# MILVLG/mmnas

Hardware: AMD Instinct MI355X
Metric: supernet fwd+bwd steps/sec (VQA arch, bs=64) (higher is better)
Workload: dtype f32 (bf16x6 split-operand MFMA, fp32 accumulate); 1 GPU; Net_Search supernet WEIGHT step: sample + fwd + BCE(sum) + bwd (+ gradient all-reduce), HSIZE 256, B=64/GPU, 100x2048 regions + 14 tokens, dropout 0.1 (search_vqa.py:279-292; BASELINE configs[2]); global_batch=64, parallelism=dp1, grad_allreduce=none, rccl_ranks=1, rank_id_sum_ok=True, lstm_fallback=False, dp_rows=1, dp_buckets=3, optimizer_in_step=False, gemm_split=6, hip_force_dev_kernarg=1

## Files before the change

include/mmnas_hip.h:

```cpp
#ifndef MMNAS_HIP_H
#define MMNAS_HIP_H

#include <stddef.h>
#include <stdint.h>

#ifdef __cplusplus
extern "C" {
#endif

#define MMNAS_ABI_VERSION 1

enum {
  MMNAS_OK = 0,
  MMNAS_E_SHAPE = -1,
  MMNAS_E_ARG = -2,
  MMNAS_E_LAUNCH = -3
};

enum {
  MMNAS_F_NORM = 1,
  MMNAS_F_RESIDUAL = 2,
  MMNAS_F_MASK = 4,
  MMNAS_F_REL = 8,
  MMNAS_F_SELF = 16,
// ... 290 lines not shown
  void* arena;
  float* x_out; float* y_out;
  const float* dx_out; const float* dy_out;
  float* dx_in; float* dy_in;
  int use_side_stream, reserved;
  void* const* marks;
  int mixed, gate_width;
  const float* gate;
  float* dgate;
  const int* y_off;
  const int* y_tile_off;
  int Ny, y_ntiles;
  const int* x_off;
  int Nx, reserved3;
} mmnas_chain;
int mmnas_chain_plan(const mmnas_chain* c, size_t* arena_bytes);
int mmnas_chain_fwd(const mmnas_chain* c, void* stream);
int mmnas_chain_bwd(const mmnas_chain* c, void* stream);
int mmnas_chain_join(void* main_stream, void* waiting_stream);
int mmnas_set_chain_overlap(int on);
int mmnas_set_wgrad_live(int on);
int mmnas_wgrad_live_table_ints(int M);
int mmnas_wgrad_live_table(const float* dy, const unsigned char* mask, int M, int d, int* tab, void* stream);

typedef struct mmnas_attflat_side {
  int S, reserved;
  const float* x; const uint8_t* mask;
  const float* W1; const float* b1; const float* W2; const float* b2; const float* Wm; const float* bm;
  float* dW1; float* db1; float* dW2; float* db2; float* dWm; float* dbm;
  uint64_t seed;
  float* dx;
  const int* off;
  int M, reserved2;
} mmnas_attflat_side;
typedef struct mmnas_head {
  int B, d, MID, G, OUT, ANS, flags, reserved;
  float drop_p, eps;
  mmnas_attflat_side sx, sy;
  const float* ln_a; const float* ln_b; float* dln_a; float* dln_b;
  const float* Wp; const float* bp; float* dWp; float* dbp;
  float* logits;
  const float* dlogits;
  void* arena;
} mmnas_head;
int mmnas_head_plan(const mmnas_head* hd, size_t* arena_bytes);
int mmnas_head_fwd(const mmnas_head* hd, void* stream);
// ... 76 lines not shown
```

mmnas_amd/_lib.py:

```python
import ctypes as C
import logging
import os

import torch

from . import switches

_HERE = os.path.dirname(os.path.abspath(__file__))
LIB_PATH = os.environ.get(switches.LIB_PATH.name) or os.path.join(_HERE, 'lib', 'libmmnas_hip.so')

log = logging.getLogger('mmnas_amd')


def _launch_configuration():
    name = 'HIP_FORCE_DEV_KERNARG'
    if name in os.environ:
        return os.environ[name], 'inherited'
    if torch.cuda.is_initialized():
        log.warning('mmnas_amd was imported after HIP had initialised and %s is not set: kernel arguments go through host-visible '
                    'memory, the ~300 short launches of a step run 20-40 %% slower.  Export %s=1 or import mmnas / mmnas_amd '
                    'before the first CUDA call.', name, name)
        return None, 'unset_after_hip_init'
    os.environ[name] = '1'
    return '1', 'set_by_library'
# ... 164 lines not shown
    'mmnas_alpha_full_step_cost': (_i, [_fp] * 7 + [_i, _i, _f, _f, _f, _f, _f, _f, _f, _i, _i, _fp]),
    'mmnas_alpha_two_step_cost': (_i, [_fp] * 7 + [_i, _i, C.POINTER(C.c_int), _f, _f, _f, _f, _f, _f, _f, _i, _i, _fp]),
    'mmnas_embedding_bwd': (_i, [_fp, _fp, _fp, C.c_long, _i, C.c_long, _fp]),
    'mmnas_node_mix_fwd': (_i, [_fp, _fp, _fp, _i, _fp, _fp, _i, _i, _f, _fp]),
    'mmnas_node_mix_bwd': (_i, [_fp, _fp, _fp, _i, _fp, _fp, _fp, _i, _fp, _fp, _i, _i, _f, _fp]),
    'mmnas_node_mix_bwd_ln': (_i, [_fp, _fp, _fp, _i, _fp, _fp, _i, _fp, _fp, _fp, _fp, _fp, _fp, _fp, _fp, _f, _u64, _u32, _i, _i, _f, _fp]),
    'mmnas_embedding_bwd_det': (_i, [_fp, _fp, _fp, _fp, C.c_long, _i, C.c_long, _f, _fp]),
    'mmnas_embedding_bwd_det_ws_floats': (_sz, [C.c_long, _i]),
    'mmnas_rel_fused_supported': (_i, [_i, _i, _i]),
    'mmnas_rel_fused_fwd': (_i, [_fp, _fp, _fp, _fp, _fp, _fp, _i, _i, _i, _i, _i, _i, _fp]),
    'mmnas_rel_fused_bwd_ws_floats': (_sz, [_i, _i, _i]),
    'mmnas_rel_fused_bwd': (_i, [_fp, _fp, _fp, _fp, _fp, _fp, _fp, _fp, _fp, _fp, _fp, _i, _i, _i, _i, _i, _i, _fp]),
    'mmnas_rel_fused_fwd_ragged': (_i, [_fp, _fp, _fp, _fp, _fp, _fp, _i, _i, _i, _i, _i, _fp, _fp]),
    'mmnas_rel_fused_bwd_ragged': (_i, [_fp] * 11 + [_i, _i, _i, _i, _i, _fp, _fp, _i, _fp]),
    'mmnas_rel_multi_supported': (_i, [_i, _i, _i]),
    'mmnas_rel_multi_bwd_ws_floats': (_sz, [_i, _i]),
    'mmnas_rel_multi_fwd': (_i, [C.POINTER(RelMulti), _fp]),
    'mmnas_rel_multi_bwd': (_i, [C.POINTER(RelMulti), _fp]),
    'mmnas_set_rel_hoist': (_i, [_i]),
    'mmnas_set_rel_keylimit': (_i, [_i]),
    'mmnas_set_wgrad_live': (_i, [_i]),
    'mmnas_wgrad_live_table_ints': (_i, [_i]),
    'mmnas_wgrad_live_table': (_i, [_fp, _fp, _i, _i, _fp, _fp]),
    'mmnas_set_guided_hoist': (_i, [_i]),
    'mmnas_set_rel_overlap': (_i, [_i]),
    'mmnas_mha_core_fwd': (_i, [C.POINTER(MhaDesc), _fp]),
    'mmnas_mha_core_bwd': (_i, [C.POINTER(MhaDesc), _fp]),
    'mmnas_mha_core_fwd_indexed': (_i, [C.POINTER(MhaDesc), _fp, _fp]),
    'mmnas_itm_pair_head': (_i, [_fp] * 11 + [C.c_long, _i, _i, _f, _fp]),
    'mmnas_rank_matrix': (_i, [_fp, _i, _i, C.c_long, _fp, _fp, _fp, _fp, _fp, _fp]),
    'mmnas_row_topk': (_i, [_fp, _i, _i, C.c_long, _i, _fp, _fp, _fp]),
    'mmnas_vgd_targets': (_i, [_fp, _fp, _fp, _i, _i, C.c_double, _i, _fp, _fp, _fp, _fp, _fp, _fp, _fp]),
    'mmnas_vgd_ground': (_i, [_fp] * 5 + [_i, _i, C.c_double] + [_fp] * 7),
    'mmnas_vqa_answer': (_i, [_fp, _i, _i, C.c_long, _fp, C.c_long, _i, _i] + [_fp] * 4 + [_i] + [_fp] * 5),
    'mmnas_vqa_accuracy': (_i, [_fp] * 4 + [_i] * 4 + [_fp, _fp, _fp]),
    'mmnas_vqa_answer_targets': (_i, [_fp, _i, _i, _i, _fp, _fp, _fp]),
    'mmnas_vgd_loss_fwd': (_i, [_fp] * 6 + [_i] * 6 + [C.c_double, C.c_double] + [_fp] * 5),
    'mmnas_itm_triplet_loss_fwd': (_i, [_fp, _fp, _fp, C.c_long, _i, _f, _i, _fp, _fp, _fp]),
    'mmnas_loss_grad_scale': (_i, [_fp, _fp, _fp, _sz, _fp]),
    'mmnas_vgd_head_supported': (_i, [_i, _i]),
    'mmnas_vgd_head_bwd_ws_floats': (_sz, [_i, _i, _i]),
    'mmnas_vgd_head_fwd': (_i, [_fp] * 12 + [_i, _i, _i, _f, _i, _fp]),
    'mmnas_vgd_head_bwd': (_i, [_fp] * 20 + [_i, _i, _i, _f, _i, _fp]),
    'mmnas_att_op_plan': (_i, [C.POINTER(AttOp), C.POINTER(Plan)]),
    'mmnas_att_op_fwd': (_i, [C.POINTER(AttOp), _fp]),
    'mmnas_att_op_bwd': (_i, [C.POINTER(AttOp), _fp]),
# ... 78 lines not shown
```

mmnas_amd/csrc/ops.hip:

```cpp
#include <string.h>
#include <functional>
#include <vector>
#include "common.h"

namespace mmnas {

static inline size_t al(size_t n) { return (n + 255) & ~(size_t)255; }
template <class Op> static inline bool drops(const Op* op) { return (op->flags & MMNAS_F_TRAIN) && op->drop_p > 0.f; }

struct Carver {
  char* base; size_t off;
  explicit Carver(void* p) : base((char*)p), off(0) {}
  float* take(size_t nfloats) { float* r = (float*)(base + off); off += al(nfloats * sizeof(float)); return r; }
};

static void gemm_init(mmnas_gemm_desc& g, int layout, int N, int K, int lda, int ldb, int ldc) {
  memset(&g, 0, sizeof(g));
  g.layout = layout; g.ngroups = 1; g.nseg = 1; g.N = N; g.K = K; g.lda = lda; g.ldb = ldb; g.ldc = ldc;
  g.alpha = 1.f; g.gate_scale = 1.f; g.split_k = 1;
}

struct AttLayout {
  size_t Mq, Mk;
  float *Q, *K, *V, *att, *stats, *z, *biasT;
// ... 723 lines not shown
    b.a.xq = in; b.a.xkv = self ? in : chain_x_final(c, L);
    b.a.dy = dy; b.a.dxq = dx;
    b.a.dxkv = self ? nullptr : chain_buf(c, L.dpre);
    b.a.drel = nullptr;
  } else { b.m.x = in; b.m.dy = dy; b.m.dx = dx; }
  return dx;
}
static int chain_run_fwd(const BoundOp& b, hipStream_t s, bool defer_ln, bool* ln_done, bool rel_ready, bool kv_ready) {
  return b.att ? att_fwd_impl(&b.a, s, defer_ln, ln_done, rel_ready, kv_ready) : mlp_fwd_impl(&b.m, s, defer_ln, ln_done);
}
static int chain_run_bwd(const BoundOp& b, hipStream_t s, SideQueue* sq, bool rel_defer, bool kv_defer, const AuxReduce* ln_pre = nullptr) {
  return b.att ? att_bwd_impl(&b.a, s, sq, !(b.a.flags & MMNAS_F_SELF), rel_defer, kv_defer, ln_pre, b.ktab) : mlp_bwd_impl(&b.m, s, sq, ln_pre, b.ktab);
}
static LnPlace chain_cand_view(const BoundOp& b, const float** z, const float** la, const float** lb) {
  LnPlace p = {false, false};
  if (b.att) p = att_ln_place(&b.a);
  if (!(b.flags() & MMNAS_F_NORM) || p.fwd) { *z = b.y; *la = nullptr; *lb = nullptr; }
  else if (b.att) { *z = b.al.z; *la = b.a.ln_a; *lb = b.a.ln_b; }
  else { *z = b.ml.z; *la = b.m.ln_a; *lb = b.m.ln_b; }
  return p;
}

constexpr int LIVE_MAX_ROWS = 8192;
int sk_workspace(hipStream_t st, float** ws, size_t* ws_floats, int** cnt, int* ncnt);
typedef unsigned u32x4_t __attribute__((ext_vector_type(4)));

__global__ void __launch_bounds__(256) wgrad_live_kernel(const float* __restrict__ dy, const uint8_t* __restrict__ mask, const int M, const int d,
                                                         int* __restrict__ tab, unsigned* __restrict__ bits, const int nwords, int* __restrict__ cnt) {
  __shared__ int s_last;
  const int tid = threadIdx.x, lane = tid & 63, wave = tid >> 6;
  const int w = blockIdx.x * 4 + wave;
  if (w < nwords) {
    const int r0 = w * 32;
    const int r = r0 + (lane & 31);
    const bool in = lane < 32 && r < M;
    const bool masked = in && mask[r] != 0;
    const unsigned need = (unsigned)__ballot(masked);
    unsigned live = (unsigned)__ballot(in && !masked);
    const __amdgpu_buffer_rsrc_t rs = __builtin_amdgcn_make_buffer_rsrc((void*)dy, 0, (unsigned)M * (unsigned)d * 4u, 0x00020000);
    for (int c0 = 0; c0 < d; c0 += 256) {
      const int col = c0 + lane * 4;
#pragma unroll
      for (int hb = 0; hb < 2; ++hb) {
        u32x4_t v[16];
#pragma unroll
        for (int i = 0; i < 16; ++i) {
          const int rr = hb * 16 + i;
          const bool ld = ((need >> rr) & 1u) != 0 && col < d;
          v[i] = __builtin_amdgcn_raw_buffer_load_b128(rs, ld ? (unsigned)((r0 + rr) * d + col) * 4u : ~0u, 0, 0);
        }
#pragma unroll
        for (int i = 0; i < 16; ++i) {
          const bool nz = ((v[i].x | v[i].y | v[i].z | v[i].w) & 0x7fffffffu) != 0;
          if (__ballot(nz) != 0) live |= 1u << (hb * 16 + i);
        }
      }
    }
    if (lane == 0) __hip_atomic_store(bits + w, live, __ATOMIC_RELAXED, __HIP_MEMORY_SCOPE_AGENT);
  }
  asm volatile("s_waitcnt vmcnt(0)" ::: "memory");
  __syncthreads();
  if (tid == 0) s_last = __hip_atomic_fetch_add(cnt, 1, __ATOMIC_RELAXED, __HIP_MEMORY_SCOPE_AGENT) == (int)gridDim.x - 1;
  __syncthreads();
  if (!s_last || wave != 0) return;
  if (lane == 0) __hip_atomic_store(cnt, 0, __ATOMIC_RELAXED, __HIP_MEMORY_SCOPE_AGENT);
  unsigned wd[4];
#pragma unroll
  for (int j = 0; j < 4; ++j) {
    const int i = 2 * lane + (j & 1) + 128 * (j >> 1);
    wd[j] = i < nwords ? __hip_atomic_load(bits + i, __ATOMIC_RELAXED, __HIP_MEMORY_SCOPE_AGENT) : 0u;
  }
  int count = 0, pos = 0;
  while (pos < M) {
    const int wi = pos >> 6, sl = wi & 63;
    const unsigned lo = wi < 64 ? __builtin_amdgcn_readlane(wd[0], sl) : __builtin_amdgcn_readlane(wd[2], sl);
    const unsigned hi = wi < 64 ? __builtin_amdgcn_readlane(wd[1], sl) : __builtin_amdgcn_readlane(wd[3], sl);
    const unsigned long long m = (((unsigned long long)hi << 32) | lo) >> (pos & 63);
    if (m == 0) { pos = (wi + 1) << 6; continue; }
    const int r = pos + __builtin_ctzll(m);
    if (lane == 0) tab[1 + count] = r;
    ++count;
    pos = r + 32;
  }
  if (lane == 0) tab[0] = count;
}

static int live_table_launch(const float* dy, const uint8_t* mask, int M, int d, int* tab, hipStream_t st) {
  const int nwords = cdiv(M, 32);
  float* ws; size_t wsf; int* cnt; int ncnt;
  const int rc = sk_workspace(st, &ws, &wsf, &cnt, &ncnt);
  if (rc) return rc;
  MMNAS_LAUNCH(wgrad_live_kernel, dim3(cdiv(nwords, 4)), dim3(256), 0, st, dy, mask, M, d, tab, (unsigned*)(tab + 1 + nwords), nwords, cnt + ncnt - 1);
  return check_launch("wgrad_live_table");
}
static bool live_table_fits(long M, int d) { return M > 0 && M <= LIVE_MAX_ROWS && d > 0 && d % 4 == 0 && (double)M * d * 4.0 < 4.0e9; }

struct SideCtx { hipStream_t side; hipStream_t enc; hipEvent_t ev[MMNAS_CHAIN_MAX_OPS + 2]; hipEvent_t ovl[4]; bool used; };
static std::mutex g_side_mu;
static std::map<std::pair<int, hipStream_t>, SideCtx> g_side;

static SideCtx* side_ctx(hipStream_t main, bool create) {
  int dev = 0;
  if (hipGetDevice(&dev) != hipSuccess) return nullptr;
  std::lock_guard<std::mutex> lk(g_side_mu);
  auto key = std::make_pair(dev, main);
  auto it = g_side.find(key);
  if (it == g_side.end()) {
// ... 207 lines not shown
  return chain_rel_fwd(RG, st, 0);
}
static int chain_rel_join(SideCtx* rsc, hipStream_t st) { return ev_fork(rsc->side, st, rsc->ovl[1]); }
static int chain_fwd_passthrough(const mmnas_chain* c, const ChainLayout& L, hipStream_t st) {
  const size_t nx = chain_rows_x(c) * c->d * sizeof(float), ny = chain_rows_y(c) * c->d * sizeof(float);
  if (L.last_x < 0 && hipMemcpyAsync(c->x_out, c->x_in, nx, hipMemcpyDeviceToDevice, st) != hipSuccess) return MMNAS_E_LAUNCH;
  if (L.last_y < 0 && hipMemcpyAsync(c->y_out, c->y_in, ny, hipMemcpyDeviceToDevice, st) != hipSuccess) return MMNAS_E_LAUNCH;
  return MMNAS_OK;
}

struct ChainBwd {
  const mmnas_chain* c; const ChainLayout* L;
  hipStream_t st;
  SideQueue* sq;
  RelGroups RG;
  GuidedSet GS;
  int G;
  float *dpre, *encdy;
  size_t ex;
  const float* enc_grad = nullptr;
  SideCtx* rel_bwd_side = nullptr;
  const int* ktab = nullptr;
};
static int chain_live_table(const mmnas_chain* c, const ChainLayout& L, hipStream_t st, const int** out) {
  *out = nullptr;
  if (!c->y_mask || c->y_off || L.first_y < 0 || !sw::wgrad_live.get() || !live_table_fits((long)c->B * c->Sy, c->d)) return MMNAS_OK;
  int* tab = (int*)chain_buf(c, L.ktab);
  const int rc = live_table_launch(c->dy_out, c->y_mask, c->B * c->Sy, c->d, tab, st);
  if (!rc) *out = tab;
  return rc;
}
static int chain_bwd_begin(ChainBwd& S, const mmnas_chain* c, const ChainLayout& L, hipStream_t st, SideQueue* sq, bool hoist) {
  S.c = c; S.L = &L; S.st = st; S.sq = sq;
  S.dpre = chain_buf(c, L.dpre); S.encdy = chain_buf(c, L.encdy);
  S.ex = chain_rows_x(c) * c->d;
  if (int r = chain_live_table(c, L, st, &S.ktab)) return r;
  if (hoist) chain_rel_groups(c, L, true, S.RG);
  chain_guided_set(c, true, hoist, S.GS);
  S.G = -1;
  for (int i = 0; i < c->n_ops && S.G < 0; ++i)
    if (S.GS.hoisted[i]) S.G = i;
  if (L.n_guided > S.GS.n && hipMemsetAsync(S.dpre, 0, S.ex * sizeof(float), st) != hipSuccess) return MMNAS_E_LAUNCH;
  return MMNAS_OK;
}
static int chain_enc_dy(ChainBwd& S, hipStream_t s, const float** out) {
  const mmnas_chain* c = S.c;
  MMNAS_REQUIRE(c->dx_out || S.L->n_guided, MMNAS_E_ARG, "chain_bwd: no gradient reaches the encoder (dx_out NULL, no guided operator)");
  if (S.enc_grad) { *out = S.enc_grad; return MMNAS_OK; }
  if (c->dx_out && S.L->n_guided) {
    const int r = mmnas_drop_add(c->dx_out, S.dpre, S.encdy, S.ex, 0.f, 0, 0, s);
// ... 292 lines not shown
    SideCtx* oc = side_ctx(st, true);
    MMNAS_REQUIRE(oc, MMNAS_E_LAUNCH, "chain_bwd: cannot create the encoder stream");
    for (int i = c->n_ops - 1; i >= G; --i)
      if ((rc = run(i, st, cur_dy, &cur_dy))) return rc;
    if ((rc = ev_fork(st, oc->enc, oc->ovl[2]))) return rc;
    const float* enc_dy = nullptr;
    if ((rc = chain_enc_dy(S, oc->enc, &enc_dy))) return rc;
    int ie = L.last_x, id = G - 1;
    while (ie >= L.first_x || id >= L.first_y) {
      if (ie >= L.first_x && (rc = run(ie--, oc->enc, enc_dy, &enc_dy))) return rc;
      if (id >= L.first_y && (rc = run(id--, st, cur_dy, &cur_dy))) return rc;
    }
    if ((rc = ev_fork(oc->enc, st, oc->ovl[3]))) return rc;
    if (c->marks)
      for (int i = 0; i < c->n_ops; ++i)
        if (c->marks[i] && hipEventRecord((hipEvent_t)c->marks[i], st) != hipSuccess) {
          set_error("chain_bwd: cannot record the mark event of operator %d", i);
          return MMNAS_E_LAUNCH;
        }
  }
  return chain_bwd_close(S, nullptr);
}

extern "C" int mmnas_chain_join(void* main_stream, void* waiting_stream) {
  SideCtx* sc = side_ctx((hipStream_t)main_stream, false);
  if (!sc || !sc->used) return MMNAS_OK;
  hipEvent_t e = sc->ev[MMNAS_CHAIN_MAX_OPS];
  if (hipEventRecord(e, sc->side) != hipSuccess || hipStreamWaitEvent((hipStream_t)waiting_stream, e, 0) != hipSuccess) {
    set_error("chain_join: event record / wait failed");
    return MMNAS_E_LAUNCH;
  }
  return MMNAS_OK;
}

namespace mmnas {

struct HeadSideLayout { float *h, *logit, *probs, *pooled, *dpooled, *dlog, *dh, *dxpool, *g1part; };
static inline int head_rows(const mmnas_head* hd, const mmnas_attflat_side& sd) { return sd.off ? sd.M : hd->B * sd.S; }
struct HeadLayout {
  HeadSideLayout s[2];
  float *xo, *sum, *xy, *dxy, *dsum, *lnws, *g1proj, *dlogT;
  size_t total;
};

static HeadLayout head_layout(const mmnas_head* hd) {
  HeadLayout L;
// ... 189 lines not shown
```

mmnas_amd/csrc/switches.h:

```cpp
#pragma once

namespace mmnas {

int env_int(const char* name, int dflt);

enum SwKind { sw_int, sw_bool, sw_exact1, sw_presence, sw_string };
enum SwPolicy { sw_once, sw_every_call, sw_reload };

struct Switch {
  const char* name;
  int dflt;
  SwKind kind;
  SwPolicy policy;
  const char* help;
  int value;
  int state;

  int get() { return state ? value : read(); }
  int read();
  int reload();
  int set(int v);
  int peek(int* source) const;
};

#define MMNAS_SWITCHES(X) \
   \
  X(chain_overlap, "MMNAS_CHAIN_OVERLAP", 0, bool, once, "language stream beside the leading image-stream operators (mmnas_set_chain_overlap); measured: no gain, DESIGN.md section 5") \
  X(head_overlap, "MMNAS_HEAD_OVERLAP", 0, bool, once, "the answer head's two AttFlat sides on two streams") \
  X(head_glimpse1, "MMNAS_HEAD_GLIMPSE1", 1, bool, every_call, "0: the head's one-glimpse logit layer as GEMM launches (A/B, tests); ops.py reads it too") \
  X(head_projt, "MMNAS_HEAD_PROJT", 1, bool, every_call, "0: the answer projection's gradients from the untransposed loss gradient") \
  X(rel_hoist, "MMNAS_REL_HOIST", 1, bool, once, "relation bias of all lazy-handle operators of a stream in one launch per direction (mmnas_set_rel_hoist); 0: one fused launch per operator (supernet step 4.54 -> 5.00 ms)") \
  X(rel_overlap, "MMNAS_REL_OVERLAP", 0, bool, once, "the image stream's relation launches on a second stream (mmnas_set_rel_overlap); measured slower, +2.5 % on the supernet step") \
  X(node_lnb, "MMNAS_NODE_LNB", 1, bool, once, "architecture step: the sampled candidate's LayerNorm backward inside the node's mix kernel (7.81 -> 7.72 ms, profiles/r06_node_lnb_ab.txt); 0: its own launch") \
  X(guided_hoist, "MMNAS_GUIDED_HOIST", 1, bool, once, "key / value projections of a chain's guided operators as grouped launches (mmnas_set_guided_hoist)") \
  X(rel_fwd_valu, "MMNAS_REL_FWD_VALU", 0, exact1, every_call, "1: a lone RelSelfAtt computes its bias with the per-operator fused kernel instead of the one-operator multi kernel (A/B)") \
  X(side_prio, "MMNAS_SIDE_PRIO", 1, bool, every_call, "0: the chains' extra streams without stream priorities (read when a stream pair is created)") \
  X(side_flush, "MMNAS_SIDE_FLUSH", 0, string, once, "op: side-stream parameter-gradient work released behind every operator instead of once per phase") \
  X(wgrad_live, "MMNAS_WGRAD_LIVE", 1, int, once, "image-stream weight gradients of a padded batch's chain reduce over the 32-row K-tiles that cover the live gradient rows only (mmnas_set_wgrad_live); 0: all B Sy rows") \
   \
  X(small_ops, "MMNAS_SMALL_OPS", 1, bool, once, "SelfAtt of <= 16 rows as one launch forward (mmnas_set_small_ops); 0: the general path") \
  X(small_bwd, "MMNAS_SMALL_BWD", 1, bool, once, "the same operators' backward as two launches (mmnas_set_small_bwd)") \
  X(small_ffn, "MMNAS_SMALL_FFN", 0, int, once, "FeedForward forward as one launch (mmnas_set_small_ffn): 1 four slices of 256 hidden units, 2 eight of 128; measured neutral (profiles/r05_small_ffn_ab.txt)") \
   \
  X(gemm_ln, "MMNAS_GEMM_LN", 0, exact1, once, "1: the merge / last FFN product and its LayerNorm as one row-panel launch (mmnas_set_gemm_ln); measured neutral, profiles/r06_ab.txt") \
  X(gemm_ln_minm, "MMNAS_GEMM_LN_MINM", 2048, int, once, "fewest rows for the row-panel kernel (read together with MMNAS_GEMM_LN)") \
  X(gemm_ln_maxk, "MMNAS_GEMM_LN_MAXK", 256, int, once, "largest K for the row-panel kernel (read together with MMNAS_GEMM_LN)") \
   \
  X(mha_nw, "MMNAS_MHA_NW", 4, int, every_call, "2: attention cores never use 4-wave workgroups (4-wave groups measured 7-15 % faster; the streaming forward always runs four)") \
  X(mha_stream_mink, "MMNAS_MHA_STREAM_MINK", 257, int, every_call, "fewest keys at which the attention forward streams the keys in blocks of 128 (1..257; more than 256 keys always stream; dense rows only)") \
  X(mha_pair, "MMNAS_MHA_PAIR", 1, bool, once, "0: two attention cores of one geometry as two launches (mixed chain)") \
  X(mha_bwd_fused, "MMNAS_MHA_BWD_FUSED", 1, bool, once, "0: the attention backward as separate dQ and dK / dV kernels (dense rows only)") \
  X(mha_fwd_b16, "MMNAS_MHA_FWD_B16", 1, bool, once, "0: attention forward (d_h = 64, 65..128 keys) on the fp32 MFMA kernels instead of split-bf16 operands (profiles/r06_attention_b16_ab.txt)") \
  X(mha_fwd_b16_two, "MMNAS_MHA_FWD_B16_TWO", 320, int, once, "more than this many (sample, head) pairs: the split-bf16 forward runs two per workgroup") \
  X(mha_bwd_b16, "MMNAS_MHA_BWD_B16", 1, bool, once, "0: attention backward (d_h = 64, 65..128 keys) on the fp32 MFMA kernels instead of split-bf16 operands (supernet step -1.6 % with both)") \
   \
  X(rel_multi_dbg, "MMNAS_REL_MULTI_DBG", 0, int, once, "timing experiments of a -DMMNAS_DBG_REL=1 build only (wrong results): 1 no stores, 2 no raw reloads, 4 no head-projection MFMAs") \
  X(rel_multi_wgs, "MMNAS_REL_MULTI_WGS", 3, int, once, "workgroups per CU of the multi-operator relation forward (tuning)") \
  X(rel_multi_yield, "MMNAS_REL_MULTI_YIELD", 0, int, once, "1 | 3: the multi-operator relation kernels' yield variants (tuning)") \
  X(rel_keylimit, "MMNAS_REL_KEYLIMIT", 1, int, once, "multi-operator relation kernels of a padded batch walk only the elements under keys up to each sample's last unmasked one (mmnas_set_rel_keylimit); 0: all B S^2 elements") \
  X(rel_bwd_valu, "MMNAS_REL_BWD_VALU", 1, bool, once, "0: the fused relation backward as the all-MFMA kernel (A/B)") \
   \
// ... 29 lines not shown
```

mmnas_amd/model/nets.py:

```python
import ctypes

import numpy as np
import torch
import torch.nn as nn
import torch.nn.functional as F

from .. import ops, switches, zeroterm
from ..utils.ops_adapter import OpsAdapter
from .mixed import MixedOp, sample_indices, sample_rows
from .modules import AttFlat, LayerNorm, RelHandle

OPS_ADAPTER = OpsAdapter()
LAZY_REL = switches.LAZY_REL.get()

_PRIOR = {'enc': ['self_att_64', 'feed_forward'] * 6,
          'dec': ['rel_self_att_64', 'guided_att_64', 'feed_forward'] * 6}


class _Cell(nn.Module):
    def forward(self, s, pre=None, s_mask=None, pre_mask=None, rel_embed=None):
        for node in self.dag:
            outs = [op(s, pre, s_mask, pre_mask, rel_embed) for op in node]
            s = outs[0]
            for o in outs[1:]:
# ... 281 lines not shown
            bb = ops.linear(bbox_feat, self.bboxfeat_linear.weight, self.bboxfeat_linear.bias)
            frcn_feat = torch.cat((frcn_feat, bb), dim=-1)
        if LAZY_REL:
            if hasattr(self, 'linear_x_rel'):
                x_rel_embed = RelHandle(x_rel_embed, self.linear_x_rel.weight, self.linear_x_rel.bias)
            y_rel_embed = RelHandle(y_rel_embed, self.linear_y_rel.weight, self.linear_y_rel.bias)
        else:
            if hasattr(self, 'linear_x_rel'):
                x_rel_embed = ops.linear(x_rel_embed, self.linear_x_rel.weight, self.linear_x_rel.bias, relu=True)
            y_rel_embed = ops.linear(y_rel_embed, self.linear_y_rel.weight, self.linear_y_rel.bias, relu=True)
        rg = getattr(y_mask, '_mmnas_ragged', None)
        packed = None
        native_head = self.TASK != 'vgd' and ops.chain_enabled() and frcn_feat.is_cuda
        xrg = lp.ragged if lp is not None else None
        sinks = native_head and ops._sinked((self.attflat_x.mlp.fc.linear.weight,))
        if rg is not None and sinks:
            y_pk = ops.linear(ops.pack_rows_fn(frcn_feat, rg), self.imgfeat_linear.weight, self.imgfeat_linear.bias)
            if xrg is not None:
                packed = self.backnone.chain_packed(ops.pack_rows_fn(x_in, xrg), y_pk, x_mask, y_mask, x_rel_embed, y_rel_embed, xrg)
            if packed is None:
                xrg = None
                packed = self.backnone.chain_packed(x_in, y_pk, x_mask, y_mask, x_rel_embed, y_rel_embed)
        elif xrg is not None and sinks:
            y_in = ops.linear(frcn_feat, self.imgfeat_linear.weight, self.imgfeat_linear.bias)
            packed = self.backnone.chain_packed_x(ops.pack_rows_fn(x_in, xrg), y_in, x_mask, y_mask, x_rel_embed, y_rel_embed, xrg)
            if packed is None:
                xrg = None
        else:
            xrg = None
        if packed is not None:
            x_out, y_out = packed
            hd, hp = ops.head_record(self.attflat_x, self.attflat_y, self.proj_norm, self.proj, self.training)
            if hd is not None:
                if xrg is not None:
                    out = ops.HeadFn.apply(x_out, y_out, x_mask, y_mask, hd, hp, rg, xrg)
                else:
                    out = ops.HeadFn.apply(x_out, y_out, x_mask, y_mask, hd, hp, rg)
                return torch.sigmoid(out.squeeze(-1)) if self.TASK == 'itm' else out
            if rg is not None:
                y_out = ops.unpack_rows_fn(y_out, rg, frcn_feat.shape[0], frcn_feat.shape[1])
            if xrg is not None:
                x_out = ops.unpack_rows_fn(x_out, xrg, x_mask.shape[0], x_mask.shape[-1])
        else:
            y_in = ops.linear(frcn_feat, self.imgfeat_linear.weight, self.imgfeat_linear.bias)
            x_out, y_out = self.backnone(x_in, y_in, x_mask, y_mask, x_rel_embed, y_rel_embed)
            if native_head and x_out.is_cuda:
                hd, hp = ops.head_record(self.attflat_x, self.attflat_y, self.proj_norm, self.proj, self.training)
                if hd is not None:
                    out = ops.HeadFn.apply(x_out, y_out, x_mask, y_mask, hd, hp)
                    return torch.sigmoid(out.squeeze(-1)) if self.TASK == 'itm' else out
        x_out = self.attflat_x(x_out, x_mask)
        if self.TASK == 'vgd':
            y_out = ops.linear(y_out, self.attfc_y.weight, self.attfc_y.bias)
            if ops.vgd_head_enabled() and y_out.is_cuda:
                return ops.grounding_head(y_out, x_out, self.proj_norm.a_2, self.proj_norm.b_2, self.proj_norm.eps,
                                          self.proj_scores.weight, self.proj_scores.bias, self.proj_reg.weight,
                                          self.proj_reg.bias, log_softmax=C.SCORES_LOSS == 'kld')
            xy = self.proj_norm(x_out.unsqueeze(1) + y_out)
            scores = ops.linear(xy, self.proj_scores.weight, self.proj_scores.bias).squeeze(-1)
            if C.SCORES_LOSS == 'kld':
                scores = F.log_softmax(scores, dim=-1)
            return scores, ops.linear(xy, self.proj_reg.weight, self.proj_reg.bias)
        y_out = self.attflat_y(y_out, y_mask)
        xy = self.proj_norm(x_out + y_out)
        out = ops.linear(xy, self.proj.weight, self.proj.bias)
        if self.TASK == 'itm':
            return torch.sigmoid(out.squeeze(-1))
# ... 206 lines not shown
```

mmnas_amd/ops.py:

```python
import ctypes as C
import math
import os
import threading

import torch

from . import _lib as L
from . import switches as S

_seed_lock = threading.Lock()
_seed_state = {'base': None, 'counter': 0}


def manual_seed(seed):
    with _seed_lock:
        _seed_state['base'] = int(seed) & 0xFFFFFFFFFFFFFFFF
        _seed_state['counter'] = 0


def next_seed():
    with _seed_lock:
        if _seed_state['base'] is None:
            _seed_state['base'] = int(torch.initial_seed()) & 0xFFFFFFFFFFFFFFFF
        _seed_state['counter'] += 1
# ... 355 lines not shown
            gg.A[s] = L.fptr(grp['A'][s])
            gg.B[s] = L.ptr(grp['B'][s]) if b_planes else L.fptr(grp['B'][s])
        gg.C = L.fptr(grp['C'])
        gg.bias = L.fptr(grp.get('bias'))
        gg.residual = L.fptr(grp.get('residual'))
        gg.gate = L.fptr(grp.get('gate'))
        gg.colsum = L.fptr(grp.get('colsum'))
    return g


def gemm(*args, **kw):
    g = gemm_desc(*args, **kw)
    L.check(L.lib().mmnas_gemm(C.byref(g), L.stream()))


def gemm_pair(dgrad, wgrad):
    L.check(L.lib().mmnas_gemm_pair(C.byref(dgrad), C.byref(wgrad), L.stream()))


def _glimpse1_on():
    return S.HEAD_GLIMPSE1.get()


class LinearFn(torch.autograd.Function):

    @staticmethod
    def forward(ctx, x, W, b, relu):
        ctx.params = (W, b)
        x, W = _f32c(x), _f32c(W)
        K = x.shape[-1]
        M = x.numel() // K
        N = W.shape[0]
        y = torch.empty(x.shape[:-1] + (N,), dtype=torch.float32, device=x.device)
        ctx.one = N == 1 and not relu and _glimpse1_on() and bool(L.lib().mmnas_glimpse1_supported(K))
        if ctx.one:
            L.check(L.lib().mmnas_glimpse1_fwd(L.fptr(x), L.fptr(W), L.fptr(_f32c(b) if b is not None else None), L.fptr(y), M, K,
                                               L.stream()))
        else:
            gemm(L.GEMM_NT, [dict(M=M, A=[x], B=[W], C=y, bias=(_f32c(b) if b is not None else None))],
                 N, K, K, K, N, relu=relu)
        ctx.save_for_backward(x, W, y if relu else None)
        ctx.has_bias, ctx.relu = b is not None, relu
        return y

    @staticmethod
    def backward(ctx, dy):
        x, W, y = ctx.saved_tensors
        dy = _f32c(dy)
        K = x.shape[-1]
        M = x.numel() // K
        N = W.shape[0]
        if ctx.relu:
            dy = torch.ops.aten.threshold_backward(dy, y, 0.0)
        (dW, db), rets, sinks = _grad_bufs(ctx.params, x.device)
        if ctx.one:
            dx = torch.empty_like(x)
            ws = _ws_floats(L.lib().mmnas_glimpse1_bwd_ws_floats(M, K), x.device)
            L.check(L.lib().mmnas_glimpse1_bwd(L.fptr(dy), L.fptr(x), L.fptr(W), L.fptr(dx), L.fptr(dW),
                                               L.fptr(db if ctx.has_bias else None), L.fptr(ws), M, K, L.stream()))
            for sk in sinks:
                sk.done()
            return (dx if ctx.needs_input_grad[0] else None), rets[0], rets[1], None
        wgrad = gemm_desc(L.GEMM_TN, [dict(M=N, A=[dy], B=[x], C=dW)], K, M, N, K, K, accumulate=True)
        dx = None
        if ctx.needs_input_grad[0]:
            dx = torch.empty_like(x)
            gemm_pair(gemm_desc(L.GEMM_NN, [dict(M=M, A=[dy], B=[W], C=dx)], K, N, N, K, K), wgrad)
        else:
            L.check(L.lib().mmnas_gemm(C.byref(wgrad), L.stream()))
        if ctx.has_bias:
            L.check(L.lib().mmnas_colsum(L.fptr(dy), L.fptr(db), M, N, N, L.stream()))
        for sk in sinks:
            sk.done()
        return dx, rets[0], rets[1], None


class EmbeddingFn(torch.autograd.Function):

    @staticmethod
    def forward(ctx, idx, weight):
        ctx.weight = weight
        ctx.save_for_backward(idx)
        ctx.rows_key = None
        s = getattr(weight, '_mmnas_sink', None)
        rows = getattr(s.owner, 'row_exchange', None) if s is not None and s.owner is not None else None
        if rows is not None and rows.active and rows.i == s.index and weight.grad is s.view and _sinks_on[0] and ctx.needs_input_grad[1]:
            ctx.rows_key = rows.gather_indices(idx)
        return torch.nn.functional.embedding(idx, weight)

    @staticmethod
    def backward(ctx, dy):
        idx, = ctx.saved_tensors
        w = ctx.weight
        dy = _f32c(dy)
        idx = idx.contiguous()
        (dW,), rets, sinks = _grad_bufs([w], dy.device)
        rows = getattr(sinks[0].owner, 'row_exchange', None) if sinks and sinks[0].owner is not None else None
# ... 53 lines not shown
            L.check(lib.mmnas_gemm(C.byref(wg_ih), L.stream()))
        gemm(L.GEMM_TN, [dict(M=4 * H, A=[DG], B=[st[0]], C=dWhh)], H, M, 4 * H, H, H, accumulate=True)
        L.check(lib.mmnas_colsum(L.fptr(DG), L.fptr(dbih), M, 4 * H, 4 * H, L.stream()))
        L.check(lib.mmnas_colsum(L.fptr(DG), L.fptr(dbhh), M, 4 * H, 4 * H, L.stream()))
        for sk in sinks:
            sk.done()
        return dx, rets[0], rets[1], rets[2], rets[3]


def lstm(x, mod):
    return LstmFn.apply(x, mod.weight_ih_l0, mod.weight_hh_l0, mod.bias_ih_l0, mod.bias_hh_l0)


def lstm_enabled():
    return S.LSTM.get()


def lstm_supported(x, mod):
    return (x.is_cuda and x.dtype == torch.float32 and x.dim() == 3 and mod.num_layers == 1 and not mod.bidirectional
            and mod.batch_first and mod.bias and mod.proj_size == 0 and mod.input_size % 4 == 0
            and bool(L.lib().mmnas_lstm_seq_supported(mod.hidden_size, x.shape[0])))


def linear(x, W, b=None, relu=False):
    return LinearFn.apply(x, W, b, relu)


class LayerNormFn(torch.autograd.Function):

    @staticmethod
    def forward(ctx, x, a, b, eps):
        x, a, b = _f32c(x), _f32c(a), _f32c(b)
        d = x.shape[-1]
        M = x.numel() // d
        y = torch.empty_like(x)
        L.check(L.lib().mmnas_layernorm_fwd(L.fptr(x), L.fptr(a), L.fptr(b), L.fptr(y), M, d, eps, L.stream()))
        ctx.save_for_backward(x, a)
        ctx.eps = eps
        return y

    @staticmethod
    def backward(ctx, dy):
        x, a = ctx.saved_tensors
        dy = _f32c(dy)
        d = x.shape[-1]
        M = x.numel() // d
        dx = torch.empty_like(x)
        dab = torch.zeros(2, d, dtype=torch.float32, device=x.device)
# ... 716 lines not shown

    @staticmethod
    def backward(ctx, g):
        B, S, _ = ctx.shape
        return unpack_rows(_f32c(g), ctx.rg, B, S), None


def pack_rows_fn(x, rg):
    x = _f32c(x)
    if x.requires_grad and torch.is_grad_enabled():
        return _PackRowsFn.apply(x, rg)
    return pack_rows(x, rg)


class BackboneFn(torch.autograd.Function):

    @staticmethod
    def forward(ctx, x, y, x_mask, y_mask, x_rel, y_rel, records, params, op_params=None, mixed=None, ragged=None, packed_io=False,
                gviews=None, *ptensors):
        lib = L.lib()
        x_ragged = None
        if ptensors and isinstance(ptensors[-1], Ragged):
            x_ragged, ptensors = ptensors[-1], ptensors[:-1]
        x, y = _f32c(x), _f32c(y)
        if x_ragged is not None:
            B, Sx, d = len(x_ragged.lengths), int(x_mask.shape[-1]), x.shape[-1]
        else:
            B, Sx, d = x.shape
        packed_io = bool(packed_io and ragged is not None)
        Sy = int(y_mask.shape[-1]) if packed_io else y.shape[1]
        if ragged is not None and not packed_io:
            y = pack_rows(y, ragged)
        n = len(records)
        arr = (L.ChainOp * n)(*records)
        ch = L.Chain()
        ch.n_ops, ch.ops = n, arr
        ch.B, ch.Sx, ch.Sy, ch.d = B, Sx, Sy, d
        xm, ym = _mask_u8(x_mask, B, Sx), _mask_u8(y_mask, B, Sy)
        xr = _f32c(x_rel) if x_rel is not None else None
        yr = _f32c(y_rel) if y_rel is not None else None
        ch.x_in, ch.y_in, ch.x_mask, ch.y_mask = L.fptr(x), L.fptr(y), L.ptr(xm), L.ptr(ym)
        ch.x_rel, ch.y_rel = L.fptr(xr), L.fptr(yr)
        if mixed is not None:
            ch.mixed, ch.gate, ch.dgate, ch.gate_width = 1, mixed[0], mixed[1], mixed[2]
        if ragged is not None:
            ch.y_off, ch.y_tile_off, ch.Ny, ch.y_ntiles = L.ptr(ragged.off), L.ptr(ragged.tile_off), ragged.N, ragged.ntiles
# ... 28 lines not shown
        dx_out = _f32c(dx_out) if dx_out is not None else None
        ragged, B, Sy, packed_io = ctx.ragged
        if packed_io:
            dy_out = _f32c(dy_out) if dy_out is not None else torch.zeros_like(y_out)
        elif ragged is not None:
            dy_out = pack_rows(_f32c(dy_out), ragged) if dy_out is not None else torch.zeros_like(y_out)
        else:
            dy_out = _f32c(dy_out) if dy_out is not None else torch.zeros_like(y_out)
        dx_in, dy_in = torch.empty_like(x), torch.empty_like(y)
        ch.dx_out, ch.dy_out, ch.dx_in, ch.dy_in = L.fptr(dx_out), L.fptr(dy_out), L.fptr(dx_in), L.fptr(dy_in)
        side = side_stream_enabled() if ctx.gviews is None else 0
        ch.use_side_stream = int(side)
        marks = marr = None
        owner = getattr(getattr(params[0], '_mmnas_sink', None), 'owner', None) if (params and ctx.gviews is None) else None
        if owner is not None and ctx.op_params is not None and not side and _last_live(ctx, params):
            marks = owner.chain_marks(ctx.op_params)
        if marks is not None:
            marr = (C.c_void_p * len(marks))(*[(ev.cuda_event if ev is not None else None) for ev in marks])
            ch.marks = C.cast(marr, C.c_void_p)
        else:
            ch.marks = None
        L.check(lib.mmnas_chain_bwd(C.byref(ch), L.stream()))
        ch.marks = None
        ctx.keep = None
        if side:
            _side_pending.append((arena, x, y, xm, ym, xr, yr, x_out, y_out, dx_out, dy_out, arr))
            if not _side_join_queued[0]:
                _side_join_queued[0] = True
                torch.autograd.Variable._execution_engine.queue_callback(join_side_stream)
        if ctx.gviews is None:
            _release_sinks(ctx, params)
        if ragged is not None and not packed_io:
            dy_in = unpack_rows(dy_in, ragged, B, Sy)
        head = (dx_in, dy_in, None, None, None, None, None, None, None, None, None, None, None)
        if ctx.gviews is not None:
            gv, ctx.gviews = ctx.gviews, None
            return head + tuple(gv) + (None,)
        return head + (None,) * (ctx.n_extra + 1)


def backbone_chain(x, y, x_mask, y_mask, x_rel, y_rel, records, params, op_params=None, mixed=None, ragged=None, packed_io=False,
                   gviews=None, ptensors=(), x_ragged=None):
    if x_ragged is not None:
        return BackboneFn.apply(x, y, x_mask, y_mask, x_rel, y_rel, records, params, op_params, mixed, ragged, packed_io, gviews, *ptensors,
                                x_ragged)
    return BackboneFn.apply(x, y, x_mask, y_mask, x_rel, y_rel, records, params, op_params, mixed, ragged, packed_io, gviews, *ptensors)
# ... 369 lines not shown
```

Baseline: 243.8 steps/s.

## Reuse chain live-row table for image stem weight gradient and parallelize table build

The image stem linear layer's weight gradient now reuses the live-row K-tile table the backbone chain builds during backward. Its reduction then covers only the 32-row tiles holding live gradient rows of the padded image batch, not all B*Sy rows. The final pass of the live-table kernel is also rewritten: a serial single-wave walk becomes a 256-thread block walk using per-word chain starts and a ballot/prefix compaction. The cost is extra Python plumbing to hand the table and its arena from the chain's backward to the linear's backward, plus a harder-to-verify table-building algorithm.

Measured after the change: 245.6 steps/s (median of 6 runs). Within noise of the previous version (+0.7%).

```diff
diff --git a/include/mmnas_hip.h b/include/mmnas_hip.h
--- a/include/mmnas_hip.h
+++ b/include/mmnas_hip.h
@@ -336,6 +336,7 @@
 int mmnas_set_wgrad_live(int on);
 int mmnas_wgrad_live_table_ints(int M);
 int mmnas_wgrad_live_table(const float* dy, const unsigned char* mask, int M, int d, int* tab, void* stream);
+const int* mmnas_chain_live_table(const mmnas_chain* c);
 
 typedef struct mmnas_attflat_side {
   int S, reserved;
diff --git a/mmnas_amd/_lib.py b/mmnas_amd/_lib.py
--- a/mmnas_amd/_lib.py
+++ b/mmnas_amd/_lib.py
@@ -210,6 +210,7 @@
     'mmnas_set_wgrad_live': (_i, [_i]),
     'mmnas_wgrad_live_table_ints': (_i, [_i]),
     'mmnas_wgrad_live_table': (_i, [_fp, _fp, _i, _i, _fp, _fp]),
+    'mmnas_chain_live_table': (_fp, [C.POINTER(Chain)]),
     'mmnas_set_guided_hoist': (_i, [_i]),
     'mmnas_set_rel_overlap': (_i, [_i]),
     'mmnas_mha_core_fwd': (_i, [C.POINTER(MhaDesc), _fp]),
diff --git a/mmnas_amd/csrc/ops.hip b/mmnas_amd/csrc/ops.hip
--- a/mmnas_amd/csrc/ops.hip
+++ b/mmnas_amd/csrc/ops.hip
@@ -769,11 +769,13 @@
 }
 
 constexpr int LIVE_MAX_ROWS = 8192;
+constexpr int LIVE_WORDS = LIVE_MAX_ROWS / 32;
 int sk_workspace(hipStream_t st, float** ws, size_t* ws_floats, int** cnt, int* ncnt);
 typedef unsigned u32x4_t __attribute__((ext_vector_type(4)));
 
 __global__ void __launch_bounds__(256) wgrad_live_kernel(const float* __restrict__ dy, const uint8_t* __restrict__ mask, const int M, const int d,
                                                          int* __restrict__ tab, unsigned* __restrict__ bits, const int nwords, int* __restrict__ cnt) {
+  static_assert(LIVE_WORDS == 256, "the walk gives every bit word one thread of the 256");
   __shared__ int s_last;
   const int tid = threadIdx.x, lane = tid & 63, wave = tid >> 6;
   const int w = blockIdx.x * 4 + wave;
@@ -809,27 +811,44 @@
   __syncthreads();
   if (tid == 0) s_last = __hip_atomic_fetch_add(cnt, 1, __ATOMIC_RELAXED, __HIP_MEMORY_SCOPE_AGENT) == (int)gridDim.x - 1;
   __syncthreads();
-  if (!s_last || wave != 0) return;
-  if (lane == 0) __hip_atomic_store(cnt, 0, __ATOMIC_RELAXED, __HIP_MEMORY_SCOPE_AGENT);
-  unsigned wd[4];
+  if (!s_last) return;
+  __shared__ uint2 s_wh[LIVE_WORDS + 2];
+  __shared__ int s_start[LIVE_WORDS];
+  __shared__ int s_nw[4];
+  if (tid == 0) __hip_atomic_store(cnt, 0, __ATOMIC_RELAXED, __HIP_MEMORY_SCOPE_AGENT);
+  const unsigned cur = tid < nwords ? __hip_atomic_load(bits + tid, __ATOMIC_RELAXED, __HIP_MEMORY_SCOPE_AGENT) : 0u;
+  const unsigned prev = tid > 0 && tid < nwords ? __hip_atomic_load(bits + tid - 1, __ATOMIC_RELAXED, __HIP_MEMORY_SCOPE_AGENT) : 0u;
+  unsigned long long y = (((unsigned long long)cur << 32) | prev) << 1;
+  y |= y << 1; y |= y << 2; y |= y << 4; y |= y << 8;
+  y |= y << 15;
+  const unsigned hard = cur & ~(unsigned)(y >> 32);
+  s_wh[tid] = make_uint2(cur, hard);
+  if (tid < 2) s_wh[LIVE_WORDS + tid] = make_uint2(0u, 0u);
+  s_start[tid] = -1;
+  __syncthreads();
+  if (hard != 0) {
+    int r = tid * 32 + __builtin_ctz(hard);
+    for (;;) {
+      s_start[r >> 5] = r;
+      const int wi = (r >> 5) + 1, sh = r & 31;
+      const uint2 e0 = s_wh[wi], e1 = s_wh[wi + 1];
+      const unsigned long long m = ((((unsigned long long)e1.x << 32) | e0.x) >> sh) << sh;
+      if (m == 0) break;
+      const int b = __builtin_ctzll(m);
+      if (((((unsigned long long)e1.y << 32) | e0.y) >> b) & 1ull) break;
+      r = wi * 32 + b;
+    }
+  }
+  __syncthreads();
+  const int st = s_start[tid];
+  const unsigned long long have = __ballot(st >= 0);
+  if (lane == 0) s_nw[wave] = __popcll(have);
+  __syncthreads();
+  int base = 0, total = 0;
 #pragma unroll
-  for (int j = 0; j < 4; ++j) {
-    const int i = 2 * lane + (j & 1) + 128 * (j >> 1);
-    wd[j] = i < nwords ? __hip_atomic_load(bits + i, __ATOMIC_RELAXED, __HIP_MEMORY_SCOPE_AGENT) : 0u;
-  }
-  int count = 0, pos = 0;
-  while (pos < M) {
-    const int wi = pos >> 6, sl = wi & 63;
-    const unsigned lo = wi < 64 ? __builtin_amdgcn_readlane(wd[0], sl) : __builtin_amdgcn_readlane(wd[2], sl);
-    const unsigned hi = wi < 64 ? __builtin_amdgcn_readlane(wd[1], sl) : __builtin_amdgcn_readlane(wd[3], sl);
-    const unsigned long long m = (((unsigned long long)hi << 32) | lo) >> (pos & 63);
-    if (m == 0) { pos = (wi + 1) << 6; continue; }
-    const int r = pos + __builtin_ctzll(m);
-    if (lane == 0) tab[1 + count] = r;
-    ++count;
-    pos = r + 32;
-  }
-  if (lane == 0) tab[0] = count;
+  for (int j = 0; j < 4; ++j) { const int n = s_nw[j]; if (j < wave) base += n; total += n; }
+  if (st >= 0) tab[1 + base + __popcll(have & ((1ull << lane) - 1ull))] = st;
+  if (tid == 0) tab[0] = total;
 }
 
 static int live_table_launch(const float* dy, const uint8_t* mask, int M, int d, int* tab, hipStream_t st) {
@@ -1083,10 +1102,14 @@
   SideCtx* rel_bwd_side = nullptr;
   const int* ktab = nullptr;
 };
+static int* chain_live_table_at(const mmnas_chain* c, const ChainLayout& L) {
+  if (!c->y_mask || c->y_off || L.first_y < 0 || !sw::wgrad_live.get() || !live_table_fits((long)c->B * c->Sy, c->d)) return nullptr;
+  return (int*)chain_buf(c, L.ktab);
+}
 static int chain_live_table(const mmnas_chain* c, const ChainLayout& L, hipStream_t st, const int** out) {
   *out = nullptr;
-  if (!c->y_mask || c->y_off || L.first_y < 0 || !sw::wgrad_live.get() || !live_table_fits((long)c->B * c->Sy, c->d)) return MMNAS_OK;
-  int* tab = (int*)chain_buf(c, L.ktab);
+  int* tab = chain_live_table_at(c, L);
+  if (!tab) return MMNAS_OK;
   const int rc = live_table_launch(c->dy_out, c->y_mask, c->B * c->Sy, c->d, tab, st);
   if (!rc) *out = tab;
   return rc;
@@ -1425,6 +1448,12 @@
   return chain_bwd_close(S, nullptr);
 }
 
+extern "C" const int* mmnas_chain_live_table(const mmnas_chain* c) {
+  ChainLayout L;
+  if (chain_check(c, "chain_live_table") || !c->arena || chain_layout(c, L)) return nullptr;
+  return chain_live_table_at(c, L);
+}
+
 extern "C" int mmnas_chain_join(void* main_stream, void* waiting_stream) {
   SideCtx* sc = side_ctx((hipStream_t)main_stream, false);
   if (!sc || !sc->used) return MMNAS_OK;
diff --git a/mmnas_amd/csrc/switches.h b/mmnas_amd/csrc/switches.h
--- a/mmnas_amd/csrc/switches.h
+++ b/mmnas_amd/csrc/switches.h
@@ -36,7 +36,7 @@
   X(rel_fwd_valu, "MMNAS_REL_FWD_VALU", 0, exact1, every_call, "1: a lone RelSelfAtt computes its bias with the per-operator fused kernel instead of the one-operator multi kernel (A/B)") \
   X(side_prio, "MMNAS_SIDE_PRIO", 1, bool, every_call, "0: the chains' extra streams without stream priorities (read when a stream pair is created)") \
   X(side_flush, "MMNAS_SIDE_FLUSH", 0, string, once, "op: side-stream parameter-gradient work released behind every operator instead of once per phase") \
-  X(wgrad_live, "MMNAS_WGRAD_LIVE", 1, int, once, "image-stream weight gradients of a padded batch's chain reduce over the 32-row K-tiles that cover the live gradient rows only (mmnas_set_wgrad_live); 0: all B Sy rows") \
+  X(wgrad_live, "MMNAS_WGRAD_LIVE", 1, int, once, "image-stream weight gradients of a padded batch's chain reduce over the 32-row K-tiles that cover the live gradient rows only, and so does the image stem's weight gradient in front of the chain (mmnas_set_wgrad_live); 0: all B Sy rows") \
    \
   X(small_ops, "MMNAS_SMALL_OPS", 1, bool, once, "SelfAtt of <= 16 rows as one launch forward (mmnas_set_small_ops); 0: the general path") \
   X(small_bwd, "MMNAS_SMALL_BWD", 1, bool, once, "the same operators' backward as two launches (mmnas_set_small_bwd)") \
diff --git a/mmnas_amd/model/nets.py b/mmnas_amd/model/nets.py
--- a/mmnas_amd/model/nets.py
+++ b/mmnas_amd/model/nets.py
@@ -327,7 +327,7 @@
                 xrg = None
                 packed = self.backnone.chain_packed(x_in, y_pk, x_mask, y_mask, x_rel_embed, y_rel_embed)
         elif xrg is not None and sinks:
-            y_in = ops.linear(frcn_feat, self.imgfeat_linear.weight, self.imgfeat_linear.bias)
+            y_in = ops.linear(frcn_feat, self.imgfeat_linear.weight, self.imgfeat_linear.bias, live=True)
             packed = self.backnone.chain_packed_x(ops.pack_rows_fn(x_in, xrg), y_in, x_mask, y_mask, x_rel_embed, y_rel_embed, xrg)
             if packed is None:
                 xrg = None
@@ -347,7 +347,7 @@
             if xrg is not None:
                 x_out = ops.unpack_rows_fn(x_out, xrg, x_mask.shape[0], x_mask.shape[-1])
         else:
-            y_in = ops.linear(frcn_feat, self.imgfeat_linear.weight, self.imgfeat_linear.bias)
+            y_in = ops.linear(frcn_feat, self.imgfeat_linear.weight, self.imgfeat_linear.bias, live=True)
             x_out, y_out = self.backnone(x_in, y_in, x_mask, y_mask, x_rel_embed, y_rel_embed)
             if native_head and x_out.is_cuda:
                 hd, hp = ops.head_record(self.attflat_x, self.attflat_y, self.proj_norm, self.proj, self.training)
diff --git a/mmnas_amd/ops.py b/mmnas_amd/ops.py
--- a/mmnas_amd/ops.py
+++ b/mmnas_amd/ops.py
@@ -401,11 +401,31 @@
     return S.HEAD_GLIMPSE1.get()
 
 
+class LiveRows:
+    __slots__ = ('tab', 'rows', 'keep')
+
+    def __init__(self):
+        self.tab = self.rows = self.keep = None
+
+    def put(self, tab, rows, keep):
+        self.tab, self.rows, self.keep = tab, rows, keep
+        torch.autograd.Variable._execution_engine.queue_callback(self.drop)
+
+    def take(self, rows):
+        got = (self.tab, self.keep) if self.tab and self.rows == rows else (None, None)
+        self.drop()
+        return got
+
+    def drop(self):
+        self.tab = self.rows = self.keep = None
+
+
 class LinearFn(torch.autograd.Function):
 
     @staticmethod
-    def forward(ctx, x, W, b, relu):
+    def forward(ctx, x, W, b, relu, live=None):
         ctx.params = (W, b)
+        ctx.live = live
         x, W = _f32c(x), _f32c(W)
         K = x.shape[-1]
         M = x.numel() // K
@@ -439,8 +459,11 @@
                                                L.fptr(db if ctx.has_bias else None), L.fptr(ws), M, K, L.stream()))
             for sk in sinks:
                 sk.done()
-            return (dx if ctx.needs_input_grad[0] else None), rets[0], rets[1], None
+            return (dx if ctx.needs_input_grad[0] else None), rets[0], rets[1], None, None
         wgrad = gemm_desc(L.GEMM_TN, [dict(M=N, A=[dy], B=[x], C=dW)], K, M, N, K, K, accumulate=True)
+        tab, arena = ctx.live.take(M) if ctx.live is not None else (None, None)
+        if tab:
+            wgrad.ktab = tab
         dx = None
         if ctx.needs_input_grad[0]:
             dx = torch.empty_like(x)
@@ -451,7 +474,8 @@
             L.check(L.lib().mmnas_colsum(L.fptr(dy), L.fptr(db), M, N, N, L.stream()))
         for sk in sinks:
             sk.done()
-        return dx, rets[0], rets[1], None
+        del arena
+        return dx, rets[0], rets[1], None, None
 
 
 class EmbeddingFn(torch.autograd.Function):
@@ -551,8 +575,13 @@
             and bool(L.lib().mmnas_lstm_seq_supported(mod.hidden_size, x.shape[0])))
 
 
-def linear(x, W, b=None, relu=False):
-    return LinearFn.apply(x, W, b, relu)
+def linear(x, W, b=None, relu=False, live=False):
+    if not (live and torch.is_grad_enabled() and x.is_cuda):
+        return LinearFn.apply(x, W, b, relu)
+    rows = LiveRows()
+    y = LinearFn.apply(x, W, b, relu, rows)
+    y._mmnas_live = rows
+    return y
 
 
 class LayerNormFn(torch.autograd.Function):
@@ -1315,6 +1344,7 @@
         x_ragged = None
         if ptensors and isinstance(ptensors[-1], Ragged):
             x_ragged, ptensors = ptensors[-1], ptensors[:-1]
+        ctx.live = getattr(y, '_mmnas_live', None) if ragged is None else None
         x, y = _f32c(x), _f32c(y)
         if x_ragged is not None:
             B, Sx, d = len(x_ragged.lengths), int(x_mask.shape[-1]), x.shape[-1]
@@ -1389,6 +1419,11 @@
             ch.marks = None
         L.check(lib.mmnas_chain_bwd(C.byref(ch), L.stream()))
         ch.marks = None
+        if ctx.live is not None:
+            tab = lib.mmnas_chain_live_table(C.byref(ch))
+            if tab:
+                ctx.live.put(tab, ch.B * ch.Sy, arena)
+            ctx.live = None
         ctx.keep = None
         if side:
             _side_pending.append((arena, x, y, xm, ym, xr, yr, x_out, y_out, dx_out, dy_out, arr))
```
